# Sienna12321/MSHA--GNN

Measured on AMD Instinct MI355X. Metric: edges/sec GAT fwd+bwd @1 GPU; link-score pairs/sec; achieved HBM GB/s vs peak, higher is better.
Workload: dtype f32; 1 GPU; gat_layer_syn100k; nodes=100000, cols=100000, edges=2000000, in_features=128, heads=8, feat=16, parallelism=replicas1

## Files before the change

### msha--gnn_amd/build.py

```python
from __future__ import annotations

import concurrent.futures as cf
import glob
import os
import subprocess
import sys

PKG = os.path.dirname(os.path.abspath(__file__))
ROOT = os.path.dirname(PKG)
CSRC = os.path.join(PKG, "csrc")
INCLUDE = os.path.join(ROOT, "include")
LIBDIR = os.path.join(PKG, "lib")
VARIANTS = {"": [], "timeline": ["-DSK_TIMELINE"],
            "nopf": ["-DGL_PREFETCH_F32=0", "-DGL_PREFETCH_BF16=0", "-DGL_EPL_F32=2"],
            "bipg16": ["-DBIP_GRP_BYTES=16384"]}
OBJDIR = os.path.join(LIBDIR, "obj")
LIB = os.path.join(LIBDIR, "libmsha_gnn.so")
ARCH = os.environ.get("MSHA_OFFLOAD_ARCH", "gfx950")
HIPCC = os.environ.get("HIPCC", "/opt/rocm/bin/hipcc")

CFLAGS = ["-O3", "-fPIC", "-std=c++17", f"--offload-arch={ARCH}", "-I", INCLUDE,
          "-Wall", "-Wno-unused-function", "-Wno-unused-variable", "-Wno-unused-parameter",
          "-fvisibility=hidden", "-munsafe-fp-atomics"]


def _headers():
    return glob.glob(os.path.join(CSRC, "*.h")) + glob.glob(os.path.join(INCLUDE, "*.h"))


def _stale(target, deps):
    if not os.path.exists(target):
        return True
    t = os.path.getmtime(target)
    return any(os.path.getmtime(d) > t for d in deps)


def _compile(src, objdir=OBJDIR, defines=()):
    obj = os.path.join(objdir, os.path.basename(src).replace(".hip", ".o"))
    if not _stale(obj, [src] + _headers()):
        return obj, None
    cmd = [HIPCC, *CFLAGS, *defines, "-c", src, "-o", obj + ".tmp"]
    r = subprocess.run(cmd, capture_output=True, text=True)
    if r.returncode != 0:
        return obj, f"$ {' '.join(cmd)}\n{r.stdout}\n{r.stderr}"
    os.replace(obj + ".tmp", obj)
    return obj, None


def build(force: bool = False, jobs: int | None = None, variant: str = "") -> str:
    defines = VARIANTS[variant]
    objdir = OBJDIR + (f"_{variant}" if variant else "")
    lib = LIB.replace(".so", f"_{variant}.so") if variant else LIB
    os.makedirs(objdir, exist_ok=True)
    srcs = sorted(glob.glob(os.path.join(CSRC, "*.hip")))
    if force:
        for o in glob.glob(os.path.join(objdir, "*.o")):
            os.remove(o)
    jobs = jobs or min(len(srcs), max(1, (os.cpu_count() or 4)), 16)
    with cf.ThreadPoolExecutor(jobs) as ex:
        results = list(ex.map(lambda src: _compile(src, objdir, defines), srcs))
    errs = [e for _, e in results if e]
    if errs:
        raise RuntimeError("hipcc failed:\n" + "\n".join(errs))
    objs = [o for o, _ in results]
    if force or _stale(lib, objs):
        cmd = [HIPCC, f"--offload-arch={ARCH}", "-shared", "-fPIC", *objs, "-o", lib + ".tmp"]
        r = subprocess.run(cmd, capture_output=True, text=True)
        if r.returncode != 0:
            raise RuntimeError(f"link failed:\n$ {' '.join(cmd)}\n{r.stdout}\n{r.stderr}")
        os.replace(lib + ".tmp", lib)
    return lib


if __name__ == "__main__":
    v = sys.argv[sys.argv.index("--variant") + 1] if "--variant" in sys.argv else ""
    print(build(force="--force" in sys.argv, variant=v))
```

### msha--gnn_amd/csrc/edge_attention.hip

```cpp
#include <stdlib.h>

#include <cstdlib>

#include "common.h"
#include "edge_geo.h"

#ifndef COLS_EH
#define COLS_EH 1
#endif
#ifndef DE_SLOT_MIN_BYTES
#define DE_SLOT_MIN_BYTES (192ll << 20)
#endif
#ifndef COLS_WIDE_UG
#define COLS_WIDE_UG 4
#endif
#ifndef COLS_EPI_BUF
#define COLS_EPI_BUF 1
#endif
#ifndef COLS_NARROW_UG
#define COLS_NARROW_UG 8
#endif
#ifndef COLS_NG
#define COLS_NG 2
#endif
// ... 561 lines not shown
        }
      }
    }
    if (G::EPI > 1) {
#pragma unroll
      for (int o = G::NQ; o < 64; o <<= 1) acc[0] = pk_xor_add(acc[0], o);
    }
#pragma unroll
    for (int k = 0; k < G::QPL; ++k) {
      if (g_e != 0) continue;
      const int q = quad_of<G>(lane, k);
      if (whole) {
        pk_store(out + (int64_t)jc * G::D + G::V * q, acc[k]);
      } else {
        float* dst = part + c * G::D + G::V * q;
#pragma unroll
        for (int i = 0; i < G::V; i += 4)
          *reinterpret_cast<float4*>(dst + i) =
              make_float4(acc[k].v[i], acc[k].v[i + 1], acc[k].v[i + 2], acc[k].v[i + 3]);
      }
    }
    if (HASX) {
      xacc = wave_xor_sum<H>(xacc);
      if (lane < H) (whole ? out_x + (int64_t)jc * H : part_x + c * H)[lane] = xacc;
    }
  }
}

constexpr int kCombineWaves = 16;

template <typename T>
__global__ void __launch_bounds__(1024) csc_combine_kernel(
    const int32_t* __restrict__ multi_col, const int32_t* __restrict__ multi_first,
    const int32_t* __restrict__ multi_count, int64_t n_multi, int D, int H,
    const float* __restrict__ part, const float* __restrict__ part_x, T* __restrict__ out,
    float* __restrict__ out_x) {
  __shared__ float red[kCombineWaves][256];
  const int W = D + (part_x != nullptr ? H : 0);
  const int64_t mi = blockIdx.x;
  const int e0 = blockIdx.y * 256;
  const int lane = threadIdx.x & 63, g = threadIdx.x >> 6;
  const int32_t jc = multi_col[mi], first = multi_first[mi], cnt = multi_count[mi];
  float acc[4] = {0.f, 0.f, 0.f, 0.f};
  auto ld = [&](int64_t c, int q) {
    const int e = e0 + lane + 64 * q;
    return e < D ? part[c * D + e] : (e < W ? part_x[c * H + (e - D)] : 0.f);
  };
  int k = g;
  for (; k + 3 * kCombineWaves < cnt; k += 4 * kCombineWaves) {
    float v[4][4];
#pragma unroll
    for (int u = 0; u < 4; ++u)
#pragma unroll
      for (int q = 0; q < 4; ++q) v[u][q] = ld(first + k + u * kCombineWaves, q);
#pragma unroll
    for (int u = 0; u < 4; ++u)
#pragma unroll
      for (int q = 0; q < 4; ++q) acc[q] += v[u][q];
  }
  for (; k < cnt; k += kCombineWaves) {
#pragma unroll
    for (int q = 0; q < 4; ++q) acc[q] += ld(first + k, q);
  }
#pragma unroll
  for (int q = 0; q < 4; ++q) red[g][lane + 64 * q] = acc[q];
  __syncthreads();
  for (int w = kCombineWaves / 2; w >= 1; w >>= 1) {
    if (g < w) {
#pragma unroll
      for (int q = 0; q < 4; ++q) red[g][lane + 64 * q] += red[g + w][lane + 64 * q];
    }
    __syncthreads();
  }
  if (g == 0) {
#pragma unroll
    for (int q = 0; q < 4; ++q) {
      const int e = e0 + lane + 64 * q;
      if (e < D) out[(int64_t)jc * D + e] = from_f32<T>(red[0][lane + 64 * q]);
      else if (e < W) out_x[(int64_t)jc * H + (e - D)] = red[0][lane + 64 * q];
    }
  }
}

#ifndef REC_PAD
#define REC_PAD 1
#endif
__host__ __device__ constexpr int rec_stride(int H) {
  int s = 1;
  while (s < 3 * H) s <<= 1;
  return REC_PAD ? s : 3 * H;
}
__host__ __device__ constexpr bool rec_has_flag(int H) { return rec_stride(H) > 3 * H; }

template <int H, int F, typename T, bool RT = false>
__global__ void __launch_bounds__(256) bwd_row_stats_kernel(
    int64_t n_rows, const float* __restrict__ el, const float* __restrict__ lse,
    const T* __restrict__ u, const T* __restrict__ u_lo, const T* __restrict__ dU,
    float* __restrict__ rec, const float* __restrict__ uc, const float* __restrict__ qc,
    const uint8_t* __restrict__ rowflag, float* __restrict__ d_el) {
  using G = Geo<H, F, T>;
  constexpr int UNR = G::QPL == 1 ? 4 : 1;
  constexpr int RPW = G::EPI * UNR;
  const int lane = lane_id();
  const int r_s = G::QPL == 1 ? lane / G::NQ : 0;
  const int64_t wave = ((int64_t)blockIdx.x * blockDim.x + threadIdx.x) >> 6;
  const int64_t nwaves = ((int64_t)gridDim.x * blockDim.x) >> 6;
  for (int64_t r0 = wave * RPW; r0 < n_rows; r0 += nwaves * RPW) {
    Pk<T> a[UNR][G::QPL], b[UNR][G::QPL];
    float4 c[UNR][G::QPL][RT ? G::V / 4 : 1];
    float elv[UNR][G::QPL], lsev[UNR][G::QPL], qcv[UNR][G::QPL];
    uint8_t fl[UNR];
    const bool lo = sizeof(T) == 2 && u_lo != nullptr;
#pragma unroll
    for (int g = 0; g < UNR; ++g) {
      const int64_t row = min(r0 + g * G::EPI + r_s, n_rows - 1);
#pragma unroll
      for (int k = 0; k < G::QPL; ++k) {
        const int q = quad_of<G>(lane, k);
        a[g][k] = pk_load(dU + row * G::D + G::V * q);
        b[g][k] = pk_load(u + row * G::D + G::V * q);
      }
#pragma unroll
      for (int k = 0; k < G::QPL; ++k) {
        const int q = quad_of<G>(lane, k);
        if (RT) {
#pragma unroll
          for (int v = 0; v < G::V / 4; ++v)
            c[g][k][v] = *reinterpret_cast<const float4*>(uc + row * G::D + G::V * q + 4 * v);
          qcv[g][k] = qc[row * H + q / G::QH];
        }
        elv[g][k] = el[row * H + q / G::QH];
        lsev[g][k] = lse[row * H + q / G::QH];
      }
      fl[g] = rowflag != nullptr ? rowflag[row] : (uint8_t)0;
    }
#pragma unroll
    for (int g = 0; g < UNR; ++g) {
      const int64_t row = r0 + g * G::EPI + r_s;
#pragma unroll
      for (int k = 0; k < G::QPL; ++k) {
        const int q = quad_of<G>(lane, k);
        float dot = pk_dot(a[g][k], b[g][k]);
        if (lo) {
          const int64_t rr = min(row, n_rows - 1);
          dot += pk_dot(a[g][k], pk_load(u_lo + rr * G::D + G::V * q));
        }
        const float dk = group_sum<G::QH>(dot);
        float dc = 0.f;
        if (RT) {
          float cv = 0.f;
#pragma unroll
          for (int v = G::V - 4; v >= 0; v -= 4) {
            const float4 c4 = c[g][k][v / 4];
            cv = fmaf(a[g][k].v[v + 3], c4.w, cv);
            cv = fmaf(a[g][k].v[v + 2], c4.z, cv);
            cv = fmaf(a[g][k].v[v + 1], c4.y, cv);
            cv = fmaf(a[g][k].v[v], c4.x, cv);
          }
          dc = group_sum<G::QH>(cv);
        }
        if (q % G::QH == 0 && row < n_rows) {
          const int h = q / G::QH;
          float* r = rec + row * rec_stride(H);
          r[h] = elv[g][k];
          r[H + h] = lsev[g][k];
          r[2 * H + h] = dk;
          const bool virt = fl[g] != 0;
          if (rec_has_flag(H) && h == 0) r[3 * H] = virt ? 1.f : 0.f;
          if (RT) d_el[row * H + h] = virt ? 0.f : fmaf(-dk, qcv[g][k], dc);
        }
      }
    }
  }
}

template <int H, int F, typename T, bool BUF, bool RSC = false>
__global__ void __launch_bounds__(256) bwd_cols_kernel(
    const int32_t* __restrict__ chunk_col, const int32_t* __restrict__ chunk_start,
    const int32_t* __restrict__ chunk_end, int64_t n_chunks, const int32_t* __restrict__ colptr,
    const int32_t* __restrict__ csc_row, const int32_t* __restrict__ csc_eid, int64_t n_rows,
    const uint8_t* __restrict__ rowflag, const float* __restrict__ rec,
    const float* __restrict__ er, const float* __restrict__ ar, const T* __restrict__ hc,
    const T* __restrict__ dU, float slope, Dropout dp, bool slot_de, float* __restrict__ de,
    T* __restrict__ d_hc, float* __restrict__ d_er, float* __restrict__ part,
    float* __restrict__ part_x) {
  using G = Geo<H, F, T>;
  const int lane = lane_id();
  const int e_s = lane / H, h_s = lane % H;
  const int g_e = G::QPL == 1 ? lane / G::NQ : 0;
  const int dsrc_k = (h_s * G::QH) / 64;
  const int dsrc_l = (h_s * G::QH) % 64;
  const int64_t wave = ((int64_t)blockIdx.x * blockDim.x + threadIdx.x) >> 6;
  const int64_t nwaves = ((int64_t)gridDim.x * blockDim.x) >> 6;

  int64_t c = wave;
  if (c >= n_chunks) return;
  int32_t jc = chunk_col[c], s0 = chunk_start[c], s1 = chunk_end[c];
  int32_t i0 = s0 + e_s < s1 ? csc_row[s0 + e_s] : 0;
  int32_t i1 = s0 + G::CE + e_s < s1 ? csc_row[s0 + G::CE + e_s] : 0;
  while (true) {
    const int64_t nc = c + nwaves;
    const bool has_next = nc < n_chunks;
    const int32_t njc = has_next ? chunk_col[nc] : 0;
    const int32_t ns0 = has_next ? chunk_start[nc] : 0;
    const int32_t ns1 = has_next ? chunk_end[nc] : 0;
    const bool whole = s0 == colptr[jc] && s1 == colptr[jc + 1];
    Pk<T> hcq[G::QPL], acc[G::QPL];
#pragma unroll
    for (int k = 0; k < G::QPL; ++k) {
      hcq[k] = pk_load(hc + (int64_t)jc * G::D + G::V * quad_of<G>(lane, k));
      acc[k] = pk_zero<T>();
    }
    float erh;
    if (RSC && G::QPL == 1) {
      const int q = lane % G::NQ;
      Pk<T> aq;
#pragma unroll
      for (int v = 0; v < G::V; ++v) aq.v[v] = ar[G::V * q + v];
      erh = __shfl(group_sum<G::QH>(pk_dot(hcq[0], aq)), h_s * G::QH);
    } else {
      erh = er[(int64_t)jc * H + h_s];
    }
    float xacc = 0.f;
    for (int32_t cs = s0; cs < s1; cs += G::CE) {
      const int32_t slot = cs + e_s;
      const bool valid = slot < s1;
      const int32_t i = i0;
      const int64_t eid = valid ? (int64_t)csc_eid[slot] : 0;
      float pre = 0.f, att = 0.f, dropf = 0.f, Dsi = 0.f;
      bool virt = false;
      if (valid) {
        const float* r = rec + (int64_t)i * rec_stride(H);
        virt = rowflag != nullptr && rowflag[i] != 0;
        pre = r[h_s] + erh;
        const float sv = virt ? 0.f : lrelu(pre, slope);
        att = __expf(sv - r[H + h_s]);
        Dsi = r[2 * H + h_s];
        dropf = dropout_factor(dp, (uint64_t)eid * H + h_s);
      }
      const float wv = att * dropf;
      const int nvalid = min(G::CE, (int)(s1 - cs));
      float gsum = 0.f;
      if constexpr (BUF && (G::EPI == 1 || COLS_EPI_BUF)) {
        constexpr int UG = G::EPI == 1 ? COLS_WIDE_UG : COLS_NARROW_UG;
        const rsrc_t r_dU = make_rsrc(dU, (uint32_t)(n_rows * G::D * sizeof(T)));
#pragma unroll
        for (int g0 = 0; g0 < G::CE; g0 += UG * G::EPI) {
          if (g0 >= nvalid) break;
          u32x4_t dl[UG][G::QPL];
#pragma unroll
          for (int u = 0; u < UG; ++u) {
            const int g = g0 + u * G::EPI;
            if (g >= G::CE) break;
            const int ei = g + g_e;
            const int32_t iq = __shfl(i, ei * H);
#pragma unroll
            for (int k = 0; k < G::QPL; ++k) {
              const int q = quad_of<G>(lane, k);
              const uint32_t off = ei < nvalid
                  ? (uint32_t)iq * (uint32_t)(G::D * sizeof(T)) + (uint32_t)(G::V * q * sizeof(T))
                  : kOOB;
              dl[u][k] = buf_b128(r_dU, off);
            }
          }
#pragma unroll
          for (int u = 0; u < UG; ++u) {
            const int g = g0 + u * G::EPI;
            if (g >= G::CE || g >= nvalid) break;
            const int ei = g + g_e;
            const bool mine = e_s >= g && e_s < g + G::EPI;
            const int srcl =
                G::QPL == 1 ? ((e_s - g) & (G::EPI - 1)) * G::NQ + h_s * G::QH : dsrc_l;
#pragma unroll
            for (int k = 0; k < G::QPL; ++k) {
              const int q = quad_of<G>(lane, k);
              const float wq = __shfl(wv, ei * H + q / G::QH);
              const Pk<T> dUi = pk_from_raw(dl[u][k], (T*)nullptr);
              acc[k] = pk_fma(wq, dUi, acc[k]);
              float t = pk_dot(dUi, hcq[k]);
              t = group_sum<G::QH>(t);
              const float cand = __shfl(t, srcl);
              if (mine && (G::QPL == 1 || k == dsrc_k)) gsum = cand;
            }
          }
        }
      } else {
#pragma unroll
      for (int g = 0; g < G::CE; g += G::EPI) {
        if (g >= nvalid) break;
        const int ei = g + g_e;
        const int32_t iq = __shfl(i, ei * H);
        const bool mine = e_s >= g && e_s < g + G::EPI;
        const int srcl = G::QPL == 1 ? ((e_s - g) & (G::EPI - 1)) * G::NQ + h_s * G::QH : dsrc_l;
#pragma unroll
        for (int k = 0; k < G::QPL; ++k) {
          const int q = quad_of<G>(lane, k);
          const float wq = __shfl(wv, ei * H + q / G::QH);
          float t = 0.f;
          if (ei < nvalid) {
            const Pk<T> dUi = pk_load(dU + (int64_t)iq * G::D + G::V * q);
            acc[k] = pk_fma(wq, dUi, acc[k]);
            t = pk_dot(dUi, hcq[k]);
          }
          t = group_sum<G::QH>(t);
          const float cand = __shfl(t, srcl);
          if (mine && (G::QPL == 1 || k == dsrc_k)) gsum = cand;
        }
      }
      }
      const int32_t sl2 = slot + 2 * G::CE;
      const int32_t i2 = sl2 < s1 ? csc_row[sl2] : 0;
      if (valid) {
        const float ds = att * (gsum * dropf - Dsi);
        const float dev = virt ? 0.f : ds * (pre > 0.f ? 1.f : slope);
        if (de != nullptr) de[(slot_de ? (int64_t)slot : eid) * H + h_s] = dev;
        xacc += dev;
      }
      i0 = i1;
      i1 = i2;
    }
    if (has_next) {
      const int32_t a0 = ns0 + e_s, a1 = ns0 + G::CE + e_s;
      i0 = a0 < ns1 ? csc_row[a0] : 0;
      i1 = a1 < ns1 ? csc_row[a1] : 0;
    }
    if (G::EPI > 1) {
#pragma unroll
      for (int o = G::NQ; o < 64; o <<= 1) acc[0] = pk_xor_add(acc[0], o);
    }
#pragma unroll
    for (int k = 0; k < G::QPL; ++k) {
      if (g_e != 0) continue;
      const int q = quad_of<G>(lane, k);
      if (whole) {
        pk_store(d_hc + (int64_t)jc * G::D + G::V * q, acc[k]);
      } else {
        float* dst = part + c * G::D + G::V * q;
#pragma unroll
        for (int v = 0; v < G::V; v += 4)
          *reinterpret_cast<float4*>(dst + v) =
              make_float4(acc[k].v[v], acc[k].v[v + 1], acc[k].v[v + 2], acc[k].v[v + 3]);
      }
    }
    xacc = wave_xor_sum<H>(xacc);
    if (lane < H) (whole ? d_er + (int64_t)jc * H : part_x + c * H)[lane] = xacc;
    if (!has_next) break;
    c = nc;
    jc = njc;
    s0 = ns0;
    s1 = ns1;
  }
}

template <int H, int F, typename T, bool RSC = false>
__global__ void __launch_bounds__(256) bwd_cols_eh_kernel(
    const int32_t* __restrict__ chunk_col, const int32_t* __restrict__ chunk_start,
    const int32_t* __restrict__ chunk_end, int64_t n_chunks, const int32_t* __restrict__ colptr,
    const int32_t* __restrict__ csc_row, const int32_t* __restrict__ csc_eid, int64_t n_edges,
    const uint8_t* __restrict__ rowflag, int64_t n_rows, const float* __restrict__ rec,
    const float* __restrict__ er, const float* __restrict__ ar, const T* __restrict__ hc,
    const T* __restrict__ dU, float slope, Dropout dp, bool slot_de, float* __restrict__ de,
    T* __restrict__ d_hc, float* __restrict__ d_er, float* __restrict__ part,
    float* __restrict__ part_x) {
  using G = Geo<H, F, T>;
  constexpr int NV = G::QH;
  constexpr int NG = COLS_NG;
  const int lane = lane_id();
  const int e_s = lane / H, h_s = lane % H;
  const int64_t wave = ((int64_t)blockIdx.x * blockDim.x + threadIdx.x) >> 6;
  const int64_t nwaves = ((int64_t)gridDim.x * blockDim.x) >> 6;
  const rsrc_t r_row = make_rsrc(csc_row, (uint32_t)(n_edges * 4));
  const rsrc_t r_eid = make_rsrc(csc_eid, (uint32_t)(n_edges * 4));
  const rsrc_t r_flag = make_rsrc(rowflag, (uint32_t)n_rows);
  const rsrc_t r_rec = make_rsrc(rec, (uint32_t)(n_rows * 4 * rec_stride(H)));
  const rsrc_t r_dU = make_rsrc(dU, (uint32_t)(n_rows * G::D * sizeof(T)));
  const rsrc_t r_de = make_rsrc(de, (uint32_t)(n_edges * 4 * H));
  const uint32_t h_off = h_s * F * sizeof(T);
  const bool need_eid = dp.active || (de != nullptr && !slot_de);

  int64_t c = wave;
  if (c >= n_chunks) return;
  int32_t jc = chunk_col[c], s0 = chunk_start[c], s1 = chunk_end[c];
  int32_t ii[NG];
#pragma unroll
  for (int g = 0; g < NG; ++g) {
    const int32_t a = s0 + g * G::CE + e_s;
    ii[g] = buf_i32(r_row, a < s1 ? (uint32_t)a * 4u : kOOB);
  }
  while (true) {
    const int64_t nc = c + nwaves;
    const bool has_next = nc < n_chunks;
    const int32_t njc = has_next ? chunk_col[nc] : 0;
    const int32_t ns0 = has_next ? chunk_start[nc] : 0;
    const int32_t ns1 = has_next ? chunk_end[nc] : 0;
    const bool whole = s0 == colptr[jc] && s1 == colptr[jc + 1];
    Pk<T> hcv[NV], acc[NV];
#pragma unroll
    for (int k = 0; k < NV; ++k) {
      hcv[k] = pk_load(hc + (int64_t)jc * G::D + h_s * F + G::V * k);
      acc[k] = pk_zero<T>();
    }
    const float er_tab = RSC ? 0.f : er[(int64_t)jc * H + h_s];
    float xacc = 0.f;
    for (int32_t cs = s0; cs < s1; cs += NG * G::CE) {
      Pk<T> dUv[NG][NV];
      int32_t eid[NG];
      float r_el[NG], r_lse[NG], Dsi[NG];
      uint32_t vflag[NG];
#pragma unroll
      for (int g = 0; g < NG; ++g) {
        const bool valid = cs + g * G::CE + e_s < s1;
        const uint32_t row_off = valid ? (uint32_t)ii[g] * (G::D * sizeof(T)) + h_off : kOOB;
#pragma unroll
        for (int k = 0; k < NV; ++k)
          dUv[g][k] = pk_load_buf(r_dU, row_off + (valid ? k * 16u : 0u), (T*)nullptr);
        eid[g] = buf_i32(r_eid, valid && need_eid ? (uint32_t)(cs + g * G::CE + e_s) * 4u : kOOB);
        const uint32_t rec_off = valid ? (uint32_t)ii[g] * (4u * rec_stride(H)) + h_s * 4u : kOOB;
        r_el[g] = buf_f32(r_rec, rec_off);
        r_lse[g] = buf_f32(r_rec, valid ? rec_off + 4u * H : kOOB);
        Dsi[g] = buf_f32(r_rec, valid ? rec_off + 8u * H : kOOB);
        if constexpr (rec_has_flag(H))
          vflag[g] = __float_as_uint(buf_f32(r_rec, valid ? rec_off - h_s * 4u + 12u * H : kOOB));
        else
          vflag[g] = buf_u8(r_flag, valid ? (uint32_t)ii[g] : kOOB);
      }
#pragma unroll
      for (int g = 0; g < NG; ++g) {
        const int32_t a = cs + (NG + g) * G::CE + e_s;
        ii[g] = buf_i32(r_row, a < s1 ? (uint32_t)a * 4u : kOOB);
      }
      float erh = er_tab;
      if (RSC) {
        Pk<T> hv[NV];
#pragma unroll
        for (int k = 0; k < NV; ++k) {
          hv[k] = hcv[k];
#pragma unroll
          for (int v = 0; v < G::V; ++v) asm volatile("" : "+v"(hv[k].v[v]));
        }
        erh = head_score<NV>(hv, ar + h_s * F);
      }
#pragma unroll
      for (int g = 0; g < NG; ++g) {
        const int32_t slot = cs + g * G::CE + e_s;
        const bool valid = slot < s1;
        const bool virt = vflag[g] != 0;
        const float pre = r_el[g] + erh;
        const float sv = virt ? 0.f : lrelu(pre, slope);
        const float att = __expf(sv - r_lse[g]);
        const float dropf = dropout_factor(dp, (uint64_t)eid[g] * H + h_s);
        const float wv = valid ? att * dropf : 0.f;
        float d[NV];
#pragma unroll
        for (int k = 0; k < NV; ++k) {
          d[k] = pk_dot(dUv[g][k], hcv[k]);
          acc[k] = pk_fma(wv, dUv[g][k], acc[k]);
        }
#pragma unroll
        for (int o = 1; o < NV; o <<= 1)
#pragma unroll
          for (int k = 0; k < NV; k += 2 * o) d[k] = d[k] + d[k + o];
        const float ds = att * (d[0] * dropf - Dsi[g]);
        const float dev = virt ? 0.f : ds * (pre > 0.f ? 1.f : slope);
#ifndef DIAG_NO_DE
        const uint32_t at = slot_de ? (uint32_t)slot : (uint32_t)eid[g];
        buf_store_f32(r_de, valid ? at * (4u * H) + h_s * 4u : kOOB, dev);
#endif
        xacc += valid ? dev : 0.f;
      }
    }
#pragma unroll
    for (int g = 0; g < NG; ++g) {
      const int32_t a = ns0 + g * G::CE + e_s;
      ii[g] = buf_i32(r_row, a < ns1 ? (uint32_t)a * 4u : kOOB);
    }
#pragma unroll
    for (int k = 0; k < NV; ++k)
#pragma unroll
      for (int o = H; o < 64; o <<= 1) acc[k] = pk_xor_add(acc[k], o);
    if (e_s == 0) {
#pragma unroll
      for (int k = 0; k < NV; ++k) {
        if (whole) {
          pk_store(d_hc + (int64_t)jc * G::D + h_s * F + G::V * k, acc[k]);
        } else {
          float* dst = part + c * G::D + h_s * F + G::V * k;
#pragma unroll
          for (int v = 0; v < G::V; v += 4)
            *reinterpret_cast<float4*>(dst + v) =
                make_float4(acc[k].v[v], acc[k].v[v + 1], acc[k].v[v + 2], acc[k].v[v + 3]);
        }
      }
    }
    xacc = wave_xor_sum<H>(xacc);
    if (lane < H) (whole ? d_er + (int64_t)jc * H : part_x + c * H)[lane] = xacc;
    if (!has_next) break;
    c = nc;
    jc = njc;
    s0 = ns0;
    s1 = ns1;
  }
}

template <int H>
__global__ void __launch_bounds__(256) bwd_row_sum_kernel(
    const int32_t* __restrict__ rowptr, int64_t n_rows, const float* __restrict__ de,
    const int32_t* __restrict__ slot_of, float* __restrict__ d_el) {
  constexpr int CE = 64 / H;
  const int lane = lane_id();
  const int r_s = lane / H, h_s = lane % H;
  const int64_t wave = ((int64_t)blockIdx.x * blockDim.x + threadIdx.x) >> 6;
  const int64_t nwaves = ((int64_t)gridDim.x * blockDim.x) >> 6;
  for (int64_t r0 = wave * CE; r0 < n_rows; r0 += nwaves * CE) {
    const int64_t row = r0 + r_s;
    if (row >= n_rows) continue;
    const int32_t start = rowptr[row], end = rowptr[row + 1];
    float p[CE];
#pragma unroll
    for (int k = 0; k < CE; ++k) p[k] = 0.f;
    for (int32_t cs = start; cs < end; cs += CE) {
      float v[CE];
      int32_t at[CE];
#pragma unroll
      for (int k = 0; k < CE; ++k)
        at[k] = slot_of == nullptr ? cs + k : (cs + k < end ? slot_of[cs + k] : 0);
#pragma unroll
      for (int k = 0; k < CE; ++k)
        v[k] = cs + k < end ? de[(int64_t)at[k] * H + h_s] : 0.f;
#pragma unroll
      for (int k = 0; k < CE; ++k)
        if (cs + k < end) p[k] += v[k];
    }
#pragma unroll
    for (int o = 1; o < CE; o <<= 1) {
#pragma unroll
      for (int k = 0; k < CE; ++k)
        if ((k & o) == 0 && (k & (2 * o - 1)) == 0) p[k] = p[k] + p[k + o];
    }
    d_el[row * H + h_s] = p[0];
  }
}

static bool shape_supported(int H, int F) {
#define X(h, f) if (H == h && F == f) return true;
  MSHA_FOR_EACH_SHAPE(X)
#undef X
  return false;
}

static int env_int(const char* name, int def) {
  const char* v = getenv(name);
  return v != nullptr && *v ? atoi(v) : def;
}

static dim3 wave_grid(int64_t items) { return dim3(grid_for(items, 4, 1 << 20)); }

static int check_graph(const msha_graph* g, bool need_csc) {
  MSHA_ARG_CHECK(g != nullptr, "graph descriptor is NULL");
  MSHA_ARG_CHECK(g->n_rows > 0 && g->n_cols > 0 && g->n_edges >= 0, "graph: bad sizes");
  MSHA_ARG_CHECK(g->rowptr && (g->n_edges == 0 || g->col), "graph: CSR arrays missing");
  if (need_csc) {
    MSHA_ARG_CHECK(g->colptr && (g->n_edges == 0 || g->csc_row), "graph: CSC arrays missing");
    MSHA_ARG_CHECK(g->n_chunks >= g->n_cols && g->chunk_col && g->chunk_start && g->chunk_end,
                   "graph: CSC chunk plan missing (need >= 1 chunk per column)");
    MSHA_ARG_CHECK(g->n_multi == 0 || (g->multi_col && g->multi_first && g->multi_count),
                   "graph: multi-chunk column list missing");
  }
  return MSHA_OK;
}

}

using namespace msha;

extern "C" int msha_edge_attention_supported(int32_t heads, int32_t feat) {
  return shape_supported(heads, feat) ? 1 : 0;
}

static bool dtype_ok(int32_t dtype, int32_t feat) {
  return dtype == MSHA_DTYPE_F32 || (dtype == MSHA_DTYPE_BF16 && feat % 8 == 0);
}

static dim3 fwd_grid(const msha_graph* g) {
  int64_t cap = env_int("MSHA_FWD_WAVES", -1);
  if (cap < 0)
    cap = g->n_edges <= (int64_t)FWD_SHORT_DEG * g->n_rows ? g->n_rows / FWD_SHORT_RPW : 0;
  return wave_grid(cap > 0 && cap < g->n_rows ? cap : g->n_rows);
}

static bool fwd_bat_ok(const msha_graph* g, int heads, int feat, int32_t dtype) {
  const int64_t lim = (int64_t)1 << 31;
  const int64_t esz = dtype == MSHA_DTYPE_BF16 ? 2 : 4;
  return env_int("MSHA_FWD_BAT", 1) != 0 && (int64_t)heads * feat * esz <= 1024 &&
         g->n_rows < lim && g->n_edges * 4 < lim && g->n_cols * 4 * heads < lim &&
         g->n_cols * heads * feat * esz < lim;
}

extern "C" int msha_edge_attention_rowterms_preferred(const msha_graph* g, int32_t heads,
                                                      int32_t feat, int32_t dtype) {
  if (g == nullptr || !shape_supported(heads, feat) || !dtype_ok(dtype, feat)) return 0;
  if (!fwd_bat_ok(g, heads, feat, dtype)) return 0;
  const int knob = env_int("MSHA_ROWTERMS", -1);
  if (knob >= 0) return knob != 0;
  if (g->n_edges * 4 * (int64_t)heads >= DE_SLOT_MIN_BYTES) return 1;
  return dtype == MSHA_DTYPE_F32 && g->n_edges >= (int64_t)FWD_SHORT_DEG * g->n_rows ? 1 : 0;
}

extern "C" int msha_edge_attention_fwd(const msha_graph* g, int32_t heads, int32_t feat,
                                       int32_t dtype, const float* el, const float* er,
                                       const void* hc, float neg_slope, float drop_p,
                                       uint64_t seed, uint64_t offset, void* u, void* u_lo,
                                       float* lse, float* attd, msha_stream_t stream) {
  return msha_edge_attention_fwd_ex(g, heads, feat, dtype, el, er, hc, neg_slope, drop_p, seed,
                                    offset, u, u_lo, lse, attd, nullptr, nullptr, stream);
}

extern "C" int msha_edge_attention_fwd_ex(const msha_graph* g, int32_t heads, int32_t feat,
                                          int32_t dtype, const float* el, const float* er,
                                          const void* hc, float neg_slope, float drop_p,
                                          uint64_t seed, uint64_t offset, void* u, void* u_lo,
                                          float* lse, float* attd, float* uc, float* qc,
                                          msha_stream_t stream) {
  if (int rc = check_graph(g, false)) return rc;
  MSHA_ARG_CHECK(el && er && hc && u && lse, "edge_attention_fwd: null pointer");
  MSHA_ARG_CHECK(drop_p >= 0.f && drop_p <= 1.f, "edge_attention_fwd: p must be in [0,1]");
  MSHA_ARG_CHECK((uc == nullptr) == (qc == nullptr), "edge_attention_fwd: uc and qc go together");
  if (!shape_supported(heads, feat) || !dtype_ok(dtype, feat))
    return fail(MSHA_ERR_UNSUPPORTED, "edge_attention_fwd: unsupported (heads, feat, dtype)");
  hipStream_t s = (hipStream_t)stream;
  const Dropout dp = make_dropout(drop_p, seed, offset, s);
  const bool bat = fwd_bat_ok(g, heads, feat, dtype);
  if (uc != nullptr && !bat)
    return fail(MSHA_ERR_UNSUPPORTED, "edge_attention_fwd: row terms need the batched forward");
  if (bat) {
    const dim3 grid = fwd_grid(g);
    const bool short_rows = g->n_edges <= (int64_t)FWD_SHORT_DEG * g->n_rows;
    if (short_rows && env_int("MSHA_FWD_GL", 1) != 0 &&
        launch_fwd_gl(g, heads, feat, dtype, el, er, nullptr, hc, neg_slope, dp, u, u_lo, lse,
// ... 127 lines not shown
    if constexpr (f % Pk<T>::V == 0) {                                                          \
      if (x)                                                                                    \
        hipLaunchKernelGGL((csc_aggregate_kernel<h, f, T, true>), wave_grid(g->n_chunks),       \
                           dim3(256), 0, s, g->chunk_col, g->chunk_start, g->chunk_end,         \
                           g->n_chunks, g->colptr, g->csc_row, g->csc_eid, w, x, ld,            \
                           (const T*)table, (T*)out, out_x, part, part_x);                      \
      else                                                                                      \
        hipLaunchKernelGGL((csc_aggregate_kernel<h, f, T, false>), wave_grid(g->n_chunks),      \
                           dim3(256), 0, s, g->chunk_col, g->chunk_start, g->chunk_end,         \
                           g->n_chunks, g->colptr, g->csc_row, g->csc_eid, w, x, ld,            \
                           (const T*)table, (T*)out, out_x, part, part_x);                      \
    }                                                                                           \
  }
  MSHA_FOR_EACH_SHAPE(X)
#undef X
  if (g->n_multi > 0) {
    const int64_t D = (int64_t)heads * feat;
    const int64_t W = D + (x ? heads : 0);
    hipLaunchKernelGGL(csc_combine_kernel<T>, dim3(g->n_multi, (W + 255) / 256),
                       dim3(64 * kCombineWaves), 0, s, g->multi_col, g->multi_first,
                       g->multi_count, g->n_multi, (int)D, heads, part, x ? part_x : nullptr,
                       (T*)out, out_x);
  }
}

extern "C" int msha_csc_aggregate(const msha_graph* g, int32_t heads, int32_t feat,
                                  int32_t dtype, const float* w, const float* x, int32_t edge_ld,
                                  const void* table, void* out, float* out_x, void* ws,
                                  size_t ws_bytes, msha_stream_t stream) {
  if (int rc = check_graph(g, true)) return rc;
  MSHA_ARG_CHECK(w && table && out, "csc_aggregate: null pointer");
  MSHA_ARG_CHECK(x == nullptr || out_x != nullptr, "csc_aggregate: x needs out_x");
  if (!shape_supported(heads, feat) || !dtype_ok(dtype, feat))
    return fail(MSHA_ERR_UNSUPPORTED, "csc_aggregate: unsupported (heads, feat, dtype)");
  const int64_t D = (int64_t)heads * feat;
  float* part = nullptr;
  float* part_x = nullptr;
  if (g->n_multi > 0) {
    MSHA_ARG_CHECK(ws != nullptr && ws_bytes >= msha_csc_aggregate_workspace_size(g, heads, feat),
                   "csc_aggregate: workspace too small");
    part = (float*)ws;
    part_x = part + g->n_chunks * D;
  }
  hipStream_t s = (hipStream_t)stream;
  const int ld = edge_ld > 0 ? edge_ld : heads;
  MSHA_ARG_CHECK(ld >= heads, "csc_aggregate: edge_ld < heads");
  if (dtype == MSHA_DTYPE_BF16)
    launch_csc<bf16_t>(g, heads, feat, w, x, ld, table, out, out_x, part, part_x, s);
  else
    launch_csc<float>(g, heads, feat, w, x, ld, table, out, out_x, part, part_x, s);
  return check_launch("csc_aggregate");
}

extern "C" size_t msha_edge_attention_bwd_fused_workspace_size(const msha_graph* g,
                                                               int32_t heads, int32_t feat) {
  if (g == nullptr || heads <= 0 || feat <= 0) return 0;
  const size_t rec = ((size_t)g->n_rows * rec_stride(heads) * sizeof(float) + 255) & ~(size_t)255;
  return rec + msha_csc_aggregate_workspace_size(g, heads, feat);
}

template <typename T>
static void launch_bwd_fused(const msha_graph* g, int heads, int feat, const float* el,
                             const float* er, const float* ar, const void* hc, const float* lse, const void* u,
                             const void* u_lo, const void* dU, float neg_slope, const Dropout& dp, float* d_el,
                             float* d_er, void* d_hc, float* de, float* rec, float* part,
                             float* part_x, const float* uc, const float* qc, hipStream_t s) {
  const bool rt = uc != nullptr;
  if (rt) de = nullptr;
  const int64_t lim = (int64_t)1 << 31;
  const bool slot_de = g->csr_slot != nullptr && g->n_edges * 4 * (int64_t)heads >= DE_SLOT_MIN_BYTES;
  const char* nobuf = getenv("MSHA_COLS_NOBUF");
  const bool buf_ok = !(nobuf != nullptr && *nobuf == '1') &&
                      g->n_rows * (int64_t)heads * feat * (int64_t)sizeof(T) < lim &&
                      g->n_edges * 4 * (int64_t)heads < lim && g->n_rows * 4 * rec_stride(heads) < lim;
#define X(h, f)                                                                                \
  if (heads == h && feat == f) {                                                               \
    if constexpr (f % Pk<T>::V == 0) {                                                         \
      auto row_stats = rt ? bwd_row_stats_kernel<h, f, T, true>                                \
                          : bwd_row_stats_kernel<h, f, T, false>;                              \
      hipLaunchKernelGGL(row_stats,                                                            \
                         wave_grid(g->n_rows / 8 + 1), dim3(256), 0, s, g->n_rows, el, lse,   \
                         (const T*)u, (const T*)u_lo, (const T*)dU, rec, uc, qc, g->rowflag,  \
                         d_el);                                                                \
      if (f * sizeof(T) <= 64 && COLS_EH && buf_ok)                                            \
        hipLaunchKernelGGL((ar != nullptr ? bwd_cols_eh_kernel<h, f, T, true>                 \
                                           : bwd_cols_eh_kernel<h, f, T, false>),               \
                           wave_grid(g->n_chunks), dim3(256), 0,                                \
                           s, g->chunk_col, g->chunk_start, g->chunk_end, g->n_chunks,         \
                           g->colptr, g->csc_row, g->csc_eid, g->n_edges, g->rowflag,          \
                           g->n_rows, rec, er, ar, (const T*)hc, (const T*)dU, neg_slope, dp,  \
                           slot_de, de,                                                        \
                           (T*)d_hc, d_er, part, part_x);                                      \
      else                                                                                     \
      {                                                                                        \
        auto kern = ar != nullptr                                                              \
            ? (buf_ok ? bwd_cols_kernel<h, f, T, true, true> : bwd_cols_kernel<h, f, T, false, true>) \
            : (buf_ok ? bwd_cols_kernel<h, f, T, true> : bwd_cols_kernel<h, f, T, false>);     \
        hipLaunchKernelGGL(kern, wave_grid(g->n_chunks), dim3(256), 0,                         \
                           s, g->chunk_col, g->chunk_start, g->chunk_end, g->n_chunks,         \
                           g->colptr, g->csc_row, g->csc_eid, g->n_rows, g->rowflag, rec, er,  \
                           ar, (const T*)hc, (const T*)dU, neg_slope, dp, slot_de,             \
                           de, (T*)d_hc, d_er,                                                 \
                           part, part_x);                                                      \
      }                                                                                        \
      if (!rt)                                                                                 \
        hipLaunchKernelGGL((bwd_row_sum_kernel<h>), wave_grid(g->n_rows), dim3(256), 0, s,     \
                           g->rowptr, g->n_rows, de, slot_de ? g->csr_slot : nullptr, d_el);  \
    }                                                                                          \
  }
  MSHA_FOR_EACH_SHAPE(X)
#undef X
  if (g->n_multi > 0) {
    const int64_t D = (int64_t)heads * feat;
    hipLaunchKernelGGL(csc_combine_kernel<T>, dim3(g->n_multi, (D + heads + 255) / 256),
                       dim3(64 * kCombineWaves), 0, s, g->multi_col, g->multi_first,
                       g->multi_count, g->n_multi, (int)D, heads, part, part_x, (T*)d_hc, d_er);
  }
}

extern "C" int msha_edge_attention_bwd_fused(const msha_graph* g, int32_t heads, int32_t feat,
                                             int32_t dtype, const float* el, const float* er,
                                             const void* hc, const float* lse, const void* u,
                                             const void* u_lo, const void* dU, float neg_slope,
                                             float drop_p,
                                             uint64_t seed, uint64_t offset, float* d_el,
                                             float* d_er, void* d_hc, float* de, void* ws,
                                             size_t ws_bytes, msha_stream_t stream) {
  return msha_edge_attention_bwd_fused_ex(g, heads, feat, dtype, el, er, hc, lse, u, u_lo, dU,
                                          neg_slope, drop_p, seed, offset, nullptr, nullptr,
                                          d_el, d_er, d_hc, de, ws, ws_bytes, stream);
}

extern "C" int msha_edge_attention_bwd_fused_ex(
    const msha_graph* g, int32_t heads, int32_t feat, int32_t dtype, const float* el,
    const float* er, const void* hc, const float* lse, const void* u, const void* u_lo,
    const void* dU, float neg_slope, float drop_p, uint64_t seed, uint64_t offset,
    const float* uc, const float* qc, float* d_el, float* d_er, void* d_hc, float* de, void* ws,
    size_t ws_bytes, msha_stream_t stream) {
  if (int rc = check_graph(g, true)) return rc;
  MSHA_ARG_CHECK(el && er && hc && lse && u && dU && d_el && d_er && d_hc,
                 "edge_attention_bwd_fused: null pointer");
  MSHA_ARG_CHECK((uc == nullptr) == (qc == nullptr), "edge_attention_bwd_fused: uc and qc go together");
  MSHA_ARG_CHECK(g->n_edges == 0 || ((de || uc) && g->csc_eid),
                 "edge_attention_bwd_fused: needs de scratch (or row terms) and csc_eid");
  MSHA_ARG_CHECK(drop_p >= 0.f && drop_p <= 1.f, "edge_attention_bwd_fused: p must be in [0,1]");
  if (!shape_supported(heads, feat) || !dtype_ok(dtype, feat))
    return fail(MSHA_ERR_UNSUPPORTED, "edge_attention_bwd_fused: unsupported (heads, feat, dtype)");
  MSHA_ARG_CHECK(ws != nullptr &&
                     ws_bytes >= msha_edge_attention_bwd_fused_workspace_size(g, heads, feat),
                 "edge_attention_bwd_fused: workspace too small");
  const int64_t D = (int64_t)heads * feat;
  float* rec = (float*)ws;
  const size_t rec_bytes = ((size_t)g->n_rows * rec_stride(heads) * sizeof(float) + 255) & ~(size_t)255;
  float* part = (float*)((char*)ws + rec_bytes);
  float* part_x = part + g->n_chunks * D;
  hipStream_t s = (hipStream_t)stream;
  const Dropout dp = make_dropout(drop_p, seed, offset, s);
  if (dtype == MSHA_DTYPE_BF16)
    launch_bwd_fused<bf16_t>(g, heads, feat, el, er, nullptr, hc, lse, u, u_lo, dU, neg_slope, dp,
                             d_el, d_er, d_hc, de, rec, part, part_x, uc, qc, s);
  else
    launch_bwd_fused<float>(g, heads, feat, el, er, nullptr, hc, lse, u, nullptr, dU, neg_slope, dp,
                            d_el, d_er, d_hc, de, rec, part, part_x, uc, qc, s);
  return check_launch("edge_attention_bwd_fused");
}

extern "C" int msha_edge_attention_row_scores_supported(const msha_graph* g, int32_t heads,
                                                        int32_t feat, int32_t dtype) {
  if (g == nullptr || !shape_supported(heads, feat) || !dtype_ok(dtype, feat)) return 0;
  return fwd_bat_ok(g, heads, feat, dtype) ? 1 : 0;
}

#ifndef RS_BF16_MIN_BYTES
#define RS_BF16_MIN_BYTES 0ll
#endif
extern "C" int msha_edge_attention_row_scores_preferred(const msha_graph* g, int32_t heads,
                                                        int32_t feat, int32_t dtype) {
  if (!msha_edge_attention_row_scores_supported(g, heads, feat, dtype)) return 0;
  const int knob = env_int("MSHA_ROW_SCORES", -1);
  if (knob >= 0) return knob != 0;
  if (dtype == MSHA_DTYPE_F32) return 1;
  return g->n_cols * 4 * (int64_t)heads >= RS_BF16_MIN_BYTES ? 1 : 0;
}
// ... 58 lines not shown
```

Measured before the change: 4.716 billion edges/s.

## Interleave per-row backward stats into float4 records and prefetch next chunk metadata

Row stats (el, lse, D, virtual flag) move from a planar layout to one interleaved float4 per (row, head). The column backward kernels can then fetch all four with a single 128-bit buffer load and no longer read a separate rowflag array. The EH column kernel also software-pipelines chunk metadata and colptr two chunks ahead, prefetches the next chunk's row indices at the end of the current inner loop, and adds a compile-time DE variant that skips de stores when de is null. The record stride grows to 4*H, and an optional environment override can cap the cols grid size.

```diff
diff --git a/msha--gnn_amd/build.py b/msha--gnn_amd/build.py
--- a/msha--gnn_amd/build.py
+++ b/msha--gnn_amd/build.py
@@ -13,7 +13,8 @@
 LIBDIR = os.path.join(PKG, "lib")
 VARIANTS = {"": [], "timeline": ["-DSK_TIMELINE"],
             "nopf": ["-DGL_PREFETCH_F32=0", "-DGL_PREFETCH_BF16=0", "-DGL_EPL_F32=2"],
-            "bipg16": ["-DBIP_GRP_BYTES=16384"]}
+            "bipg16": ["-DBIP_GRP_BYTES=16384"],
+            "colsng3": ["-DCOLS_NG=3"]}
 OBJDIR = os.path.join(LIBDIR, "obj")
 LIB = os.path.join(LIBDIR, "libmsha_gnn.so")
 ARCH = os.environ.get("MSHA_OFFLOAD_ARCH", "gfx950")
diff --git a/msha--gnn_amd/csrc/edge_attention.hip b/msha--gnn_amd/csrc/edge_attention.hip
--- a/msha--gnn_amd/csrc/edge_attention.hip
+++ b/msha--gnn_amd/csrc/edge_attention.hip
@@ -667,15 +667,7 @@
   }
 }
 
-#ifndef REC_PAD
-#define REC_PAD 1
-#endif
-__host__ __device__ constexpr int rec_stride(int H) {
-  int s = 1;
-  while (s < 3 * H) s <<= 1;
-  return REC_PAD ? s : 3 * H;
-}
-__host__ __device__ constexpr bool rec_has_flag(int H) { return rec_stride(H) > 3 * H; }
+__host__ __device__ constexpr int rec_stride(int H) { return 4 * H; }
 
 template <int H, int F, typename T, bool RT = false>
 __global__ void __launch_bounds__(256) bwd_row_stats_kernel(
@@ -746,12 +738,9 @@
         }
         if (q % G::QH == 0 && row < n_rows) {
           const int h = q / G::QH;
-          float* r = rec + row * rec_stride(H);
-          r[h] = elv[g][k];
-          r[H + h] = lsev[g][k];
-          r[2 * H + h] = dk;
           const bool virt = fl[g] != 0;
-          if (rec_has_flag(H) && h == 0) r[3 * H] = virt ? 1.f : 0.f;
+          *reinterpret_cast<float4*>(rec + (row * H + h) * 4) =
+              make_float4(elv[g][k], lsev[g][k], dk, virt ? 1.f : 0.f);
           if (RT) d_el[row * H + h] = virt ? 0.f : fmaf(-dk, qcv[g][k], dc);
         }
       }
@@ -764,7 +753,7 @@
     const int32_t* __restrict__ chunk_col, const int32_t* __restrict__ chunk_start,
     const int32_t* __restrict__ chunk_end, int64_t n_chunks, const int32_t* __restrict__ colptr,
     const int32_t* __restrict__ csc_row, const int32_t* __restrict__ csc_eid, int64_t n_rows,
-    const uint8_t* __restrict__ rowflag, const float* __restrict__ rec,
+    const float* __restrict__ rec,
     const float* __restrict__ er, const float* __restrict__ ar, const T* __restrict__ hc,
     const T* __restrict__ dU, float slope, Dropout dp, bool slot_de, float* __restrict__ de,
     T* __restrict__ d_hc, float* __restrict__ d_er, float* __restrict__ part,
@@ -815,12 +804,12 @@
       float pre = 0.f, att = 0.f, dropf = 0.f, Dsi = 0.f;
       bool virt = false;
       if (valid) {
-        const float* r = rec + (int64_t)i * rec_stride(H);
-        virt = rowflag != nullptr && rowflag[i] != 0;
-        pre = r[h_s] + erh;
+        const float4 r = *reinterpret_cast<const float4*>(rec + ((int64_t)i * H + h_s) * 4);
+        virt = r.w != 0.f;
+        pre = r.x + erh;
         const float sv = virt ? 0.f : lrelu(pre, slope);
-        att = __expf(sv - r[H + h_s]);
-        Dsi = r[2 * H + h_s];
+        att = __expf(sv - r.y);
+        Dsi = r.z;
         dropf = dropout_factor(dp, (uint64_t)eid * H + h_s);
       }
       const float wv = att * dropf;
@@ -937,12 +926,12 @@
   }
 }
 
-template <int H, int F, typename T, bool RSC = false>
+template <int H, int F, typename T, bool RSC = false, bool DE = true>
 __global__ void __launch_bounds__(256) bwd_cols_eh_kernel(
     const int32_t* __restrict__ chunk_col, const int32_t* __restrict__ chunk_start,
     const int32_t* __restrict__ chunk_end, int64_t n_chunks, const int32_t* __restrict__ colptr,
     const int32_t* __restrict__ csc_row, const int32_t* __restrict__ csc_eid, int64_t n_edges,
-    const uint8_t* __restrict__ rowflag, int64_t n_rows, const float* __restrict__ rec,
+    int64_t n_rows, const float* __restrict__ rec,
     const float* __restrict__ er, const float* __restrict__ ar, const T* __restrict__ hc,
     const T* __restrict__ dU, float slope, Dropout dp, bool slot_de, float* __restrict__ de,
     T* __restrict__ d_hc, float* __restrict__ d_er, float* __restrict__ part,
@@ -952,20 +941,27 @@
   constexpr int NG = COLS_NG;
   const int lane = lane_id();
   const int e_s = lane / H, h_s = lane % H;
-  const int64_t wave = ((int64_t)blockIdx.x * blockDim.x + threadIdx.x) >> 6;
+  const int64_t wave = __builtin_amdgcn_readfirstlane(
+      (int)(((int64_t)blockIdx.x * blockDim.x + threadIdx.x) >> 6));
   const int64_t nwaves = ((int64_t)gridDim.x * blockDim.x) >> 6;
   const rsrc_t r_row = make_rsrc(csc_row, (uint32_t)(n_edges * 4));
   const rsrc_t r_eid = make_rsrc(csc_eid, (uint32_t)(n_edges * 4));
-  const rsrc_t r_flag = make_rsrc(rowflag, (uint32_t)n_rows);
   const rsrc_t r_rec = make_rsrc(rec, (uint32_t)(n_rows * 4 * rec_stride(H)));
   const rsrc_t r_dU = make_rsrc(dU, (uint32_t)(n_rows * G::D * sizeof(T)));
-  const rsrc_t r_de = make_rsrc(de, (uint32_t)(n_edges * 4 * H));
+  const rsrc_t r_de = make_rsrc(DE ? de : nullptr, (uint32_t)(n_edges * 4 * H));
   const uint32_t h_off = h_s * F * sizeof(T);
-  const bool need_eid = dp.active || (de != nullptr && !slot_de);
+  const bool need_eid = dp.active || (DE && de != nullptr && !slot_de);
 
   int64_t c = wave;
   if (c >= n_chunks) return;
   int32_t jc = chunk_col[c], s0 = chunk_start[c], s1 = chunk_end[c];
+  int64_t nc = c + nwaves;
+  bool has_next = nc < n_chunks;
+  const int64_t ncl = has_next ? nc : c;
+  int32_t njc = chunk_col[ncl], ns0 = chunk_start[ncl];
+  const int32_t ne1 = chunk_end[ncl];
+  int32_t ns1 = has_next ? ne1 : ns0;
+  int32_t cp0 = colptr[jc], cp1 = colptr[jc + 1];
   int32_t ii[NG];
 #pragma unroll
   for (int g = 0; g < NG; ++g) {
@@ -973,12 +969,11 @@
     ii[g] = buf_i32(r_row, a < s1 ? (uint32_t)a * 4u : kOOB);
   }
   while (true) {
-    const int64_t nc = c + nwaves;
-    const bool has_next = nc < n_chunks;
-    const int32_t njc = has_next ? chunk_col[nc] : 0;
-    const int32_t ns0 = has_next ? chunk_start[nc] : 0;
-    const int32_t ns1 = has_next ? chunk_end[nc] : 0;
-    const bool whole = s0 == colptr[jc] && s1 == colptr[jc + 1];
+    const int64_t nc2 = nc + nwaves;
+    const bool has_next2 = nc2 < n_chunks;
+    const int64_t nc2l = has_next2 ? nc2 : c;
+    int32_t n2jc = chunk_col[nc2l], n2s0 = chunk_start[nc2l], n2e1 = chunk_end[nc2l];
+    int32_t ncp0 = colptr[njc], ncp1 = colptr[njc + 1];
     Pk<T> hcv[NV], acc[NV];
 #pragma unroll
     for (int k = 0; k < NV; ++k) {
@@ -990,8 +985,7 @@
     for (int32_t cs = s0; cs < s1; cs += NG * G::CE) {
       Pk<T> dUv[NG][NV];
       int32_t eid[NG];
-      float r_el[NG], r_lse[NG], Dsi[NG];
-      uint32_t vflag[NG];
+      u32x4_t rv[NG];
 #pragma unroll
       for (int g = 0; g < NG; ++g) {
         const bool valid = cs + g * G::CE + e_s < s1;
@@ -1000,19 +994,16 @@
         for (int k = 0; k < NV; ++k)
           dUv[g][k] = pk_load_buf(r_dU, row_off + (valid ? k * 16u : 0u), (T*)nullptr);
         eid[g] = buf_i32(r_eid, valid && need_eid ? (uint32_t)(cs + g * G::CE + e_s) * 4u : kOOB);
-        const uint32_t rec_off = valid ? (uint32_t)ii[g] * (4u * rec_stride(H)) + h_s * 4u : kOOB;
-        r_el[g] = buf_f32(r_rec, rec_off);
-        r_lse[g] = buf_f32(r_rec, valid ? rec_off + 4u * H : kOOB);
-        Dsi[g] = buf_f32(r_rec, valid ? rec_off + 8u * H : kOOB);
-        if constexpr (rec_has_flag(H))
-          vflag[g] = __float_as_uint(buf_f32(r_rec, valid ? rec_off - h_s * 4u + 12u * H : kOOB));
-        else
-          vflag[g] = buf_u8(r_flag, valid ? (uint32_t)ii[g] : kOOB);
-      }
-#pragma unroll
-      for (int g = 0; g < NG; ++g) {
-        const int32_t a = cs + (NG + g) * G::CE + e_s;
-        ii[g] = buf_i32(r_row, a < s1 ? (uint32_t)a * 4u : kOOB);
+        rv[g] = buf_b128(r_rec, valid ? (uint32_t)ii[g] * (4u * rec_stride(H)) + h_s * 16u : kOOB);
+      }
+      {
+        const bool last = cs + NG * G::CE >= s1;
+        const int32_t nb = last ? ns0 : cs + NG * G::CE, ne = last ? ns1 : s1;
+#pragma unroll
+        for (int g = 0; g < NG; ++g) {
+          const int32_t a = nb + g * G::CE + e_s;
+          ii[g] = buf_i32(r_row, a < ne ? (uint32_t)a * 4u : kOOB);
+        }
       }
       float erh = er_tab;
       if (RSC) {
@@ -1029,10 +1020,10 @@
       for (int g = 0; g < NG; ++g) {
         const int32_t slot = cs + g * G::CE + e_s;
         const bool valid = slot < s1;
-        const bool virt = vflag[g] != 0;
-        const float pre = r_el[g] + erh;
+        const bool virt = rv[g].w != 0;
+        const float pre = __uint_as_float(rv[g].x) + erh;
         const float sv = virt ? 0.f : lrelu(pre, slope);
-        const float att = __expf(sv - r_lse[g]);
+        const float att = __expf(sv - __uint_as_float(rv[g].y));
         const float dropf = dropout_factor(dp, (uint64_t)eid[g] * H + h_s);
         const float wv = valid ? att * dropf : 0.f;
         float d[NV];
@@ -1045,24 +1036,28 @@
         for (int o = 1; o < NV; o <<= 1)
 #pragma unroll
           for (int k = 0; k < NV; k += 2 * o) d[k] = d[k] + d[k + o];
-        const float ds = att * (d[0] * dropf - Dsi[g]);
+        const float ds = att * (d[0] * dropf - __uint_as_float(rv[g].z));
         const float dev = virt ? 0.f : ds * (pre > 0.f ? 1.f : slope);
-#ifndef DIAG_NO_DE
-        const uint32_t at = slot_de ? (uint32_t)slot : (uint32_t)eid[g];
-        buf_store_f32(r_de, valid ? at * (4u * H) + h_s * 4u : kOOB, dev);
-#endif
+        if constexpr (DE) {
+          const uint32_t at = slot_de ? (uint32_t)slot : (uint32_t)eid[g];
+          buf_store_f32(r_de, valid ? at * (4u * H) + h_s * 4u : kOOB, dev);
+        }
         xacc += valid ? dev : 0.f;
       }
-    }
-#pragma unroll
-    for (int g = 0; g < NG; ++g) {
-      const int32_t a = ns0 + g * G::CE + e_s;
-      ii[g] = buf_i32(r_row, a < ns1 ? (uint32_t)a * 4u : kOOB);
+      asm volatile("" : "+s"(n2jc), "+s"(n2s0), "+s"(n2e1), "+s"(ncp0), "+s"(ncp1));
+    }
+    if (s0 >= s1) {
+#pragma unroll
+      for (int g = 0; g < NG; ++g) {
+        const int32_t a = ns0 + g * G::CE + e_s;
+        ii[g] = buf_i32(r_row, a < ns1 ? (uint32_t)a * 4u : kOOB);
+      }
     }
 #pragma unroll
     for (int k = 0; k < NV; ++k)
 #pragma unroll
       for (int o = H; o < 64; o <<= 1) acc[k] = pk_xor_add(acc[k], o);
+    const bool whole = (s0 == cp0) & (s1 == cp1);
     if (e_s == 0) {
 #pragma unroll
       for (int k = 0; k < NV; ++k) {
@@ -1084,6 +1079,13 @@
     jc = njc;
     s0 = ns0;
     s1 = ns1;
+    cp0 = ncp0;
+    cp1 = ncp1;
+    nc = nc2;
+    has_next = has_next2;
+    njc = n2jc;
+    ns0 = n2s0;
+    ns1 = has_next2 ? n2e1 : n2s0;
   }
 }
 
@@ -1139,6 +1141,11 @@
 }
 
 static dim3 wave_grid(int64_t items) { return dim3(grid_for(items, 4, 1 << 20)); }
+
+static dim3 cols_grid(int64_t n_chunks) {
+  const int64_t waves = env_int("MSHA_COLS_WAVES", 0);
+  return wave_grid(waves > 0 && waves < n_chunks ? waves : n_chunks);
+}
 
 static int check_graph(const msha_graph* g, bool need_csc) {
   MSHA_ARG_CHECK(g != nullptr, "graph descriptor is NULL");
@@ -1432,23 +1439,30 @@
                          wave_grid(g->n_rows / 8 + 1), dim3(256), 0, s, g->n_rows, el, lse,   \
                          (const T*)u, (const T*)u_lo, (const T*)dU, rec, uc, qc, g->rowflag,  \
                          d_el);                                                                \
-      if (f * sizeof(T) <= 64 && COLS_EH && buf_ok)                                            \
-        hipLaunchKernelGGL((ar != nullptr ? bwd_cols_eh_kernel<h, f, T, true>                 \
-                                           : bwd_cols_eh_kernel<h, f, T, false>),               \
-                           wave_grid(g->n_chunks), dim3(256), 0,                                \
-                           s, g->chunk_col, g->chunk_start, g->chunk_end, g->n_chunks,         \
-                           g->colptr, g->csc_row, g->csc_eid, g->n_edges, g->rowflag,          \
+          \
+          \
+      constexpr bool narrow = f * sizeof(T) <= 64 && COLS_EH;                                  \
+      const bool eh = narrow && buf_ok;                                                        \
+      if constexpr (narrow) if (eh) {            \
+        auto kern = ar != nullptr                                                              \
+            ? (de != nullptr ? bwd_cols_eh_kernel<h, f, T, true, true>                        \
+                             : bwd_cols_eh_kernel<h, f, T, true, false>)                      \
+            : (de != nullptr ? bwd_cols_eh_kernel<h, f, T, false, true>                       \
+                             : bwd_cols_eh_kernel<h, f, T, false, false>);                    \
+        hipLaunchKernelGGL(kern, cols_grid(g->n_chunks), dim3(256),                           \
+                           0, s, g->chunk_col, g->chunk_start, g->chunk_end, g->n_chunks,      \
+                           g->colptr, g->csc_row, g->csc_eid, g->n_edges,                      \
                            g->n_rows, rec, er, ar, (const T*)hc, (const T*)dU, neg_slope, dp,  \
                            slot_de, de,                                                        \
                            (T*)d_hc, d_er, part, part_x);                                      \
-      else                                                                                     \
-      {                                                                                        \
+      }                                                                                        \
+      if (!eh) {                                                                               \
         auto kern = ar != nullptr                                                              \
             ? (buf_ok ? bwd_cols_kernel<h, f, T, true, true> : bwd_cols_kernel<h, f, T, false, true>) \
             : (buf_ok ? bwd_cols_kernel<h, f, T, true> : bwd_cols_kernel<h, f, T, false>);     \
-        hipLaunchKernelGGL(kern, wave_grid(g->n_chunks), dim3(256), 0,                         \
-                           s, g->chunk_col, g->chunk_start, g->chunk_end, g->n_chunks,         \
-                           g->colptr, g->csc_row, g->csc_eid, g->n_rows, g->rowflag, rec, er,  \
+        hipLaunchKernelGGL(kern, cols_grid(g->n_chunks), dim3(256),                           \
+                           0, s, g->chunk_col, g->chunk_start, g->chunk_end, g->n_chunks,      \
+                           g->colptr, g->csc_row, g->csc_eid, g->n_rows, rec, er,              \
                            ar, (const T*)hc, (const T*)dU, neg_slope, dp, slot_de,             \
                            de, (T*)d_hc, d_er,                                                 \
                            part, part_x);                                                      \
```

After: 4.735 billion edges/s, median of 5. Within noise of the previous version (+0.4%).
